# Mouafak-Khaled/Flow-Q-Learning

Hardware: AMD Instinct MI355X
Metric: FQL grad-steps/sec (whole node) over 16-α population, cube-single-v0 (higher is better)
Workload: dtype f32

## Files before the change

### flow-q-learning_amd/csrc/kernels.h

```cpp
#pragma once
#include <hip/hip_runtime.h>
#include <stdint.h>

namespace fq {

struct TRef {
    float* p;
    long long ss;
    long long sy;
};

inline TRef tref(float* p, long long ss, long long sy = 0) { return TRef{p, ss, sy}; }

enum GemmLayout { LAYOUT_FWD = 0, LAYOUT_DX = 1, LAYOUT_DW = 2 };
enum GemmEpi { EPI_STORE = 0, EPI_BIAS = 1, EPI_BIAS_GELU2 = 2, EPI_BIAS_GELU = 3, EPI_ADAM = 4 };

struct GemmArgs {
    TRef A, B, C, C2, bias;
    int M, N, K;
    int lda, ldb, ldc;
    int ny, nz;
    const int* slots;
    unsigned long long* probe;
};
void launch_gemm(int layout, int epi, int tile, const GemmArgs& a, hipStream_t s);
void launch_gemm_euler_hidden(const GemmArgs& a, hipStream_t s);
void launch_gemm_variant(int layout, int epi, int tile, int variant, const GemmArgs& a, hipStream_t s);
constexpr int GEMM_GROUP_MAX = 8;
struct Chunk { long long off; int len; int leaf; };
struct AdamArgs {
    const float* p_in;
    float* p_out;
    float *g, *m, *v;
    float* target;
    long long P, PT;
    long long net_off;
    const Chunk* chunks;
    const int* ids;
    int n_chunks, chunk_base;
    float* stats;
    int n_total_chunks;
    const int* count;
    float lr, tau;
    int nz;
    const int* slots;
};
struct AdamEpi {
    const float* p_in;
    float *p_out, *m, *v, *target, *wt_out;
    long long P, PT, PTT;
    long long ens, wt_sy;
    long long w_off[GEMM_GROUP_MAX];
    long long wt_off[GEMM_GROUP_MAX];
    int stat_base[GEMM_GROUP_MAX];
    float* stats;
    int n_total_chunks;
    const int* count;
    float lr, tau;
    int mode;
    int nt;
    AdamArgs small;
    int small_blocks;
};
struct GemmGroupArgs {
    GemmArgs g[GEMM_GROUP_MAX];
    int first[GEMM_GROUP_MAX + 1];
    int ng;
    AdamEpi adam;
};
void launch_gemm_group_dw(int tile, const GemmArgs* gs, int ng, hipStream_t s, const AdamEpi* adam = nullptr);
int gemm_group_tiles(int tile, int M, int N);

constexpr int EF_MAX_LAYERS = 8;
struct EulerArgs {
    const float* params;
    long long P;
    long long w_off[EF_MAX_LAYERS + 1];
    long long b_off[EF_MAX_LAYERS + 1];
    TRef eu;
    TRef aflow;
    int D, A, H, L, B, S, first;
    float steps_f;
    int nz;
    const int* slots;
    unsigned long long* probe;
    unsigned long long* phase;
};
constexpr int EF_PHASE_STRIDE = 4 * 10 * (EF_MAX_LAYERS + 1) + 8;
bool euler_flow_supported(int H, int L, int D, int A, int B);
void launch_euler_flow(const EulerArgs& a, hipStream_t s);

struct LnArgs {
    TRef u, h, mu, rstd, gamma, beta;
    int H, M, ld;
    int ny, nz;
    const int* slots;
};
void launch_ln_gelu_fwd(const LnArgs& a, hipStream_t s);

enum HeadMode { HEAD_STORE = 0, HEAD_BC_FUSED = 1, HEAD_EULER = 2, HEAD_OS = 3, HEAD_ACT = 4 };
struct HeadArgs {
    TRef h, W, b;
    TRef o0, o1, o2, o3;
    int H, M, ld, nout;
    int ld0, ld1, ld2, ld3;
    int B, D;
    int last;
    float steps_f;
    float t_next;
    int ny, nz;
    const int* slots;
};
void launch_head_fwd(int mode, const HeadArgs& a, hipStream_t s);

struct StreamArgs {
    const float* params;
    long long P, ens;
    long long w_off[EF_MAX_LAYERS + 1], b_off[EF_MAX_LAYERS + 1];
    long long g_off[EF_MAX_LAYERS], be_off[EF_MAX_LAYERS];
    const float* x0;
    long long x0_ss;
    int ld_x, K0, L, M;
    float* U[EF_MAX_LAYERS];
    float* G[EF_MAX_LAYERS];
    float* MU[EF_MAX_LAYERS];
    float* RS[EF_MAX_LAYERS];
    long long s_ss, s_sy, st_ss, st_sy;
    int ld_s, st_lo, st_hi;
    int g_hi;
    HeadArgs head;
    int ny, nz;
    const int* slots;
};
bool stream_fwd_supported(int H, int L, int K0, int nout, int M);
void launch_stream_fwd(int head_mode, bool ln, const StreamArgs& a, hipStream_t s);

struct SplitSync {
    unsigned long long* xch;
    unsigned* cnt;
    unsigned* gen;
    unsigned* err;
};
struct SplitFwdArgs {
    StreamArgs s;
    TRef aflow;
    int D, A, S, first;
    float steps_f;
    unsigned long long* probe;
    SplitSync sync;
    unsigned long long* phase;
    float* pre0;
};
long long split_cluster_bytes();
constexpr long long split_euler_pre0_floats() { return 2LL * 256 * 16; }
bool split_euler_pre0(int K0, int D);
int split_counter_stride();
bool split_fwd_supported(int H, int L, int K0, int nout, int M);
void launch_split_fwd(int head_mode, bool ln, bool euler, int F, const SplitFwdArgs& a, hipStream_t s);

struct StreamBwdArgs {
    const float* params;
    long long P, ens;
    const float* paramsT;
    long long PT, ensT;
    long long wt_off[EF_MAX_LAYERS];
    long long w_off[EF_MAX_LAYERS + 1], b_off[EF_MAX_LAYERS + 1];
    long long g_off[EF_MAX_LAYERS], be_off[EF_MAX_LAYERS];
    const float* dout;
    long long dout_ss, dout_sy;
    int ld_o;
    const float* U[EF_MAX_LAYERS];
    const float* Ghead;
    const float* MU[EF_MAX_LAYERS];
    const float* RS[EF_MAX_LAYERS];
    long long s_ss, s_sy, st_ss, st_sy;
    int ld_s, coff;
    float* DU[EF_MAX_LAYERS];
    long long d_ss, d_sy;
    int ld_d;
    float* part;
    int NP;
    int L, M, Mg, nout;
    float* da;
    long long da_ss, da_sy;
    int ld_da, D0, na;
    int ny, nz;
    const int* slots;
    unsigned long long* phase;
};
constexpr int SB_PHASE_STRIDE = 48;
bool stream_bwd_supported(int H, int L, int nout, int M, int Mg);
void launch_stream_bwd(bool ln, const StreamBwdArgs& a, hipStream_t s);
inline int stream_bwd_np(int L, int H, int nout, bool ln) { return (ln ? 3 : 1) * L * H + H * nout; }

bool split_bwd_supported(int H, int L, int nout, int M, int Mg);
void launch_split_bwd(bool ln, int F, const StreamBwdArgs& a, const SplitSync& sy, hipStream_t s);

struct ColsumArgs {
    const float* part;
    int NP, tiles;
    float* grads;
    long long P, ens;
    long long b_off[EF_MAX_LAYERS], g_off[EF_MAX_LAYERS], be_off[EF_MAX_LAYERS], w5_off;
    int L, H, ln;
    int ny, nz;
    const int* slots;
};
void launch_colsum_reduce(const ColsumArgs& a, hipStream_t s);

constexpr int TR_MAX = 32;
struct TransposeArgs {
    const float* src;
    long long src_ss;
    float* dst;
    long long dst_ss;
    long long src_off[TR_MAX], dst_off[TR_MAX];
    int n_mats, H;
    int nz;
    const int* slots;
};
void launch_transpose(const TransposeArgs& a, hipStream_t s);


struct BwdArgs {
    TRef dh;
    TRef dout, W5;
    TRef u, x_head;
    TRef mu, rstd, gamma;
    TRef c1, c2;
    TRef du;
    TRef g_b, g_gamma, g_beta, g_W5;
    int H, M, Mg, ld, ld_d, ld_o, nout;
    int ny, nz;
    const int* slots;
};
void launch_bwd_rowstats(bool head, const BwdArgs& a, hipStream_t s);
void launch_bwd_cols(bool head, bool ln, const BwdArgs& a, hipStream_t s);

struct InGradArgs {
    TRef W0, du0, da;
    int H, D, A, E, ld, off, M;
    int nz;
    const int* slots;
// ... 188 lines not shown
```

### flow-q-learning_amd/csrc/kernels.hip

```cpp
#include "kernels.h"

#include <hip/hip_runtime.h>
#include <math.h>

#include <type_traits>

#if defined(__HIP_DEVICE_COMPILE__) && !defined(__gfx950__)
#error "fqlpop kernels target gfx950 (MI355X) only: the s_waitcnt immediates use the gfx9 encoding"
#endif


namespace fq {

typedef float f32x16 __attribute__((ext_vector_type(16)));
typedef float f32x4 __attribute__((ext_vector_type(4)));

#define DEV __device__ __forceinline__

DEV float* at(TRef t, int slot, int y = 0) {
    return t.p + (long long)slot * t.ss + (long long)y * t.sy;
}

constexpr float kSqrt2OverPi = 0.7978845608028654f;

// ... 807 lines not shown
}

template <int EPI>
static void gemm_fwd_dma_dispatch(int tile, int stages, const GemmArgs& a, hipStream_t s) {
    auto grid = [&](int bm, int bn) { return dim3((a.M / bm) * (a.N / bn) * a.ny * a.nz); };
#define FQ_DMA(BM, BN, ST) hipLaunchKernelGGL((gemm_fwd_dma_kernel<BM, BN, ST, EPI>), grid(BM, BN), dim3(256), 0, s, a)
    if (tile == 0) {
        if (stages == 3) FQ_DMA(64, 64, 3);
        else FQ_DMA(64, 64, 4);
    } else if (tile == 1) {
        FQ_DMA(128, 64, 3);
    } else {
        FQ_DMA(64, 128, 3);
    }
#undef FQ_DMA
}

template <bool ARC, bool BRC, int EPI>
static void gemm_dispatch_tile(int tile, int variant, const GemmArgs& a, hipStream_t s) {
    if constexpr (!ARC && !BRC) {
        if (variant >= 4 && a.M % ((tile & 1) ? 128 : 64) == 0) {
            gemm_fwd_dma_dispatch<EPI>(tile, variant == 4 ? 3 : 4, a, s);
            return;
        }
    }
    variant &= 3;
    auto grid = [&](int bm, int bn) { return dim3(((a.M + bm - 1) / bm) * (a.N / bn) * a.ny * a.nz); };
    switch (tile) {
        case 0: gemm_dispatch_variant<64, 64, ARC, BRC, EPI>(variant, grid(64, 64), a, s); break;
        case 1: gemm_dispatch_variant<128, 64, ARC, BRC, EPI>(variant, grid(128, 64), a, s); break;
        case 2: gemm_dispatch_variant<64, 128, ARC, BRC, EPI>(variant, grid(64, 128), a, s); break;
        default: gemm_dispatch_variant<128, 128, ARC, BRC, EPI>(variant & 2, grid(128, 128), a, s); break;
    }
}

void launch_gemm_variant(int layout, int epi, int tile, int variant, const GemmArgs& a, hipStream_t s) {
    if ((tile & 2) && a.N % 128 != 0) tile &= ~2;
    if (layout != LAYOUT_FWD) variant &= 3;
    const int bk = (variant & 1) ? 64 : 32;
    if (layout != LAYOUT_FWD && a.K % bk != 0) variant &= ~1;
    if (layout == LAYOUT_FWD) {
        switch (epi) {
            case EPI_BIAS: gemm_dispatch_tile<false, false, EPI_BIAS>(tile, variant, a, s); break;
            case EPI_BIAS_GELU2: gemm_dispatch_tile<false, false, EPI_BIAS_GELU2>(tile, variant, a, s); break;
            default: gemm_dispatch_tile<false, false, EPI_BIAS_GELU>(tile, variant, a, s); break;
        }
    } else if (layout == LAYOUT_DX) {
        gemm_dispatch_tile<true, false, EPI_STORE>(tile, variant, a, s);
    } else {
        gemm_dispatch_tile<true, true, EPI_STORE>(tile, variant, a, s);
    }
}

void launch_gemm(int layout, int epi, int tile, const GemmArgs& a, hipStream_t s) {
    launch_gemm_variant(layout, epi, tile, 0, a, s);
}

void launch_gemm_euler_hidden(const GemmArgs& a, hipStream_t s) {
    const dim3 grid((a.M / 64) * (a.N / 64) * a.ny * a.nz);
    hipLaunchKernelGGL((gemm_fwd_dma_kernel<64, 64, 4, EPI_BIAS_GELU, 1>), grid, dim3(256), 0, s, a);
}

constexpr int EF_H = 512, EF_NC = 16, EF_NW = 8, EF_PF = 8, EF_K0MAX = 64;

constexpr float kG0 = -2.0f * 0.7978845608028654f * 1.4426950408889634f;
constexpr float kG1 = kG0 * 0.044715f;
DEV float gelu_sig(float x, float x2) {
    return __builtin_amdgcn_rcpf(1.0f + __builtin_amdgcn_exp2f(x * fmaf(x2, kG1, kG0)));
}
DEV float gelu_fast(float x) { return x * gelu_sig(x, x * x); }
constexpr float kD0 = 2.0f * 0.7978845608028654f, kD1 = kD0 * 3.0f * 0.044715f;
DEV void gelu_and_grad_fast(float x, float& g, float& gp) {
    const float x2 = x * x, sg = gelu_sig(x, x2);
    g = x * sg;
    gp = fmaf(sg, x * (1.0f - sg) * fmaf(x2, kD1, kD0), sg);
}
DEV float gelu_grad_fast(float x) {
    const float x2 = x * x, sg = gelu_sig(x, x2);
    return fmaf(sg, x * (1.0f - sg) * fmaf(x2, kD1, kD0), sg);
}

DEV void ln_acc(float v, float& s1, float& s2) {
#pragma clang fp contract(off)
    s1 = s1 + v;
    s2 = fmaf(v, v, s2);
}
DEV void ln_stats(float S1, float S2, float h, float& mean, float& rs) {
#pragma clang fp contract(off)
    mean = S1 / h;
    const float var = fmaxf(fmaf(-mean, mean, S2 / h), 0.f);
    rs = 1.0f / sqrtf(var + 1e-6f);
}
DEV float ln_apply(float v, float mean, float rs, float ga, float be) {
#pragma clang fp contract(off)
    return fmaf((v - mean) * rs, ga, be);
}
DEV float ln_bwd_acc(float dh, float gm, float xh, float& s1, float& s2) {
#pragma clang fp contract(off)
    const float d = dh * gm;
    s1 = s1 + d;
    s2 = fmaf(d, xh, s2);
    return d;
}
DEV float ln_bwd_du(float d, float xh, float c1, float c2, float rs, float gp) {
#pragma clang fp contract(off)
    return (rs * fmaf(-xh, c2, d - c1)) * gp;
}
DEV float mul_rn(float a, float b) {
#pragma clang fp contract(off)
    return a * b;
}

template <int PF = EF_PF>
DEV void ef_kloop(f32x4 (&acc)[4], float4 (&ring)[PF], rsrc_t rW, const float* xs, int NS, int w_cur,
                  int w_next, int lo, int lk, int li, int tail = -1) {
    constexpr int H = EF_H, NC = EF_NC;
    float bnext = xs[lk * NC + li];
    int s0 = 0;
    do {
        const int rbase = (s0 + PF < NS ? w_cur + 4 * (s0 + PF) * H : w_next) + lo;
        const int r0 = (s0 + PF >= NS && tail >= 0 ? tail : rbase - lo) + lo;
#pragma unroll
        for (int p = 0; p < PF; ++p) {
            const int s = s0 + p;
            const float b = bnext;
            bnext = xs[(4 * (s + 1) + lk) * NC + li];
            __builtin_amdgcn_sched_barrier(0);
            const float4 a = ring[p];
            acc[0] = __builtin_amdgcn_mfma_f32_16x16x4f32(a.x, b, acc[0], 0, 0, 0);
            acc[1] = __builtin_amdgcn_mfma_f32_16x16x4f32(a.y, b, acc[1], 0, 0, 0);
            acc[2] = __builtin_amdgcn_mfma_f32_16x16x4f32(a.z, b, acc[2], 0, 0, 0);
            acc[3] = __builtin_amdgcn_mfma_f32_16x16x4f32(a.w, b, acc[3], 0, 0, 0);
            __builtin_amdgcn_sched_barrier(0);
            ring[p] = bload4(rW, p == 0 ? r0 : rbase + 4 * p * H);
            __builtin_amdgcn_sched_barrier(0);
        }
        s0 += PF;
    } while (s0 < NS);
}

DEV void ef_tail(f32x4 (&acc)[4], float4 a, const float* xs, int lk, int li) {
    constexpr int NC = EF_NC;
    const float b = xs[(4 * EF_PF + lk) * NC + li];
    acc[0] = __builtin_amdgcn_mfma_f32_16x16x4f32(a.x, b, acc[0], 0, 0, 0);
    acc[1] = __builtin_amdgcn_mfma_f32_16x16x4f32(a.y, b, acc[1], 0, 0, 0);
    acc[2] = __builtin_amdgcn_mfma_f32_16x16x4f32(a.z, b, acc[2], 0, 0, 0);
    acc[3] = __builtin_amdgcn_mfma_f32_16x16x4f32(a.w, b, acc[3], 0, 0, 0);
}

bool euler_flow_supported(int H, int L, int D, int A, int B) {
    return H == EF_H && L >= 1 && L <= EF_MAX_LAYERS && D + A + 1 <= EF_K0MAX && A <= 8 && B % EF_NC == 0;
}

__global__ __launch_bounds__(EF_NW * 64, 1) void euler_flow_kernel(const EulerArgs g) {
    constexpr int H = EF_H, NC = EF_NC, NT = EF_NW * 64, PF = EF_PF;
    __shared__ __attribute__((aligned(16))) float slab[2][H * NC];
    __shared__ __attribute__((aligned(16))) float in0[EF_K0MAX * NC + 64];
    __shared__ float b5s[8];

    const int tiles = g.B / NC;
    const int total = tiles * g.nz;
    const int bid = xcd_remap(blockIdx.x, total);
    const int z = bid / tiles, c0 = (bid % tiles) * NC;
    const int slot = g.slots[z];
    const int tid = threadIdx.x, lane = tid & 63;
    const int w = __builtin_amdgcn_readfirstlane(tid >> 6);
    const int li = lane & 15, lk = lane >> 4;
    if (g.probe != nullptr && tid == 0) g.probe[2 * blockIdx.x] = __builtin_amdgcn_s_memrealtime();
#ifdef FQ_PHASE_PROBE
    unsigned long long* const ph = g.phase != nullptr ? g.phase + (long long)blockIdx.x * EF_PHASE_STRIDE : nullptr;
    auto stamp = [&](int i) {
        if (ph != nullptr && tid == 0) ph[i] = __builtin_amdgcn_s_memrealtime();
    };
#else
    auto stamp = [](int) {};
#endif
    stamp(0);

    const int D = g.D, A = g.A, L = g.L, B = g.B, S = g.S;
    const int K0 = D + A + 1;
#ifdef FQ_NO_EULER_TAIL
    const bool tail0 = false;
#else
    const bool tail0 = K0 > 4 * PF && K0 <= 4 * (PF + 1);
#endif
    const int NS0 = tail0 ? PF : (K0 + 4 * PF - 1) / (4 * PF) * PF;
    const float* __restrict__ P = g.params + (long long)slot * g.P;
    const float* __restrict__ eu = at(g.eu, slot);
    load_in0<NT>(in0, eu, D + A, B, c0);
    if (tid < A) b5s[tid] = P[g.b_off[L] + tid];
    const rsrc_t rW = make_rsrc(P, g.P);
    float w5r[16];
#pragma unroll
    for (int s = 0; s < 16; ++s) w5r[s] = bload1(rW, ((int)g.w_off[L] + (64 * w + 4 * s + lk) * A + li) * 4, 0);
#pragma unroll
    for (int s = 0; s < 16; ++s) w5r[s] = li < A ? w5r[s] : 0.f;

    const int lo = lk * H + 64 * w + 4 * li;
    float4 ring[PF];
#pragma unroll
    for (int p = 0; p < PF; ++p) ring[p] = bload4(rW, (int)g.w_off[0] + 4 * p * H + lo);
    __syncthreads();

    for (int step = g.first; step < S; ++step) {
        if (step == g.first) {
            if (tid < NC) in0[(D + A) * NC + tid] = (float)((double)step / (double)S);
            __syncthreads();
        }
        for (int l = 0; l < L; ++l) {
            const int NS = l == 0 ? NS0 : H / 4;
            const float* xs = l == 0 ? in0 : slab[(l - 1) & 1];
            float* xo = slab[l & 1];
            const int nl = l + 1 < L ? l + 1 : 0;
            f32x4 acc[4];
#pragma unroll
            for (int c = 0; c < 4; ++c) acc[c] = f32x4{0.f, 0.f, 0.f, 0.f};
            float4 bias4[4];
#pragma unroll
            for (int r = 0; r < 4; ++r) bias4[r] = bload4(rW, (int)g.b_off[l] + 64 * w + 16 * lk + 4 * r);
            __builtin_amdgcn_s_waitcnt(0x0F74);
            const int wcur = (int)g.w_off[l], wnext = (int)g.w_off[nl];
            asm volatile("" ::"s"(wcur), "s"(wnext));
            const int pi = 1 + 4 * ((step - g.first) * (L + 1) + l);
            stamp(pi);
            const bool tl = l == 0 && tail0;
            ef_kloop(acc, ring, rW, xs, NS, wcur, wnext, lo, lk, li, tl ? wcur + 4 * PF * H : -1);
            if (tl) {
                ef_tail(acc, ring[0], xs, lk, li);
                __builtin_amdgcn_sched_barrier(0);
                ring[0] = bload4(rW, wnext + lo);
            }
            stamp(pi + 1);
#pragma unroll
            for (int r = 0; r < 4; ++r) {
                const float bb[4] = {bias4[r].x, bias4[r].y, bias4[r].z, bias4[r].w};
#pragma unroll
                for (int c = 0; c < 4; ++c) {
                    const int f = 64 * w + 4 * (4 * lk + r) + c;
                    xo[f * NC + li] = gelu_fast(acc[c][r] + bb[c]);
                }
            }
            stamp(pi + 2);
            __syncthreads();
            stamp(pi + 3);
        }
        const int ph0 = 1 + 4 * ((step - g.first) * (L + 1) + L);
        stamp(ph0);
        float* red = slab[L & 1];
        {
            const float* hs = slab[(L - 1) & 1];
            f32x4 hacc = f32x4{0.f, 0.f, 0.f, 0.f};
#pragma unroll
            for (int s = 0; s < 16; ++s) {
                const int k = 64 * w + 4 * s + lk;
                hacc = __builtin_amdgcn_mfma_f32_16x16x4f32(w5r[s], hs[k * NC + li], hacc, 0, 0, 0);
            }
#pragma unroll
            for (int r = 0; r < 4; ++r) red[w * 16 * NC + (4 * lk + r) * NC + li] = hacc[r];
        }
        __syncthreads();
        if (tid < A * NC) {
            const int a = tid / NC, j = tid % NC;
            float v = red[tid];
#pragma unroll
            for (int q = 1; q < EF_NW; ++q) v += red[q * 16 * NC + tid];
            v += b5s[a];
            float* xp = &in0[(D + a) * NC + j];
            *xp = *xp + v / g.steps_f;
        } else if (tid < (A + 1) * NC && step + 1 < S) {
            in0[(D + A) * NC + tid - A * NC] = (float)((double)(step + 1) / (double)S);
        }
        __syncthreads();
        stamp(ph0 + 3);
    }
    if (tid < A * NC) {
        const int a = tid / NC, j = tid % NC;
        at(g.aflow, slot)[(long long)a * B + c0 + j] = clip1(in0[(D + a) * NC + j]);
    }
    if (g.probe != nullptr) {
        __syncthreads();
        if (tid == 0) g.probe[2 * blockIdx.x + 1] = __builtin_amdgcn_s_memrealtime();
    }
}

void launch_euler_flow(const EulerArgs& a, hipStream_t s) {
    const dim3 grid((a.B / EF_NC) * a.nz);
    hipLaunchKernelGGL(euler_flow_kernel, grid, dim3(EF_NW * 64), 0, s, a);
}

constexpr int CW = 16;

#define FQ_KPT_DISPATCH(H, KERNEL, ...)                                      \
    switch ((H) / CW) {                                                      \
        case 4: KERNEL(4, __VA_ARGS__); break;                               \
        case 8: KERNEL(8, __VA_ARGS__); break;                               \
        case 16: KERNEL(16, __VA_ARGS__); break;                             \
        case 32: KERNEL(32, __VA_ARGS__); break;                             \
        default: KERNEL(64, __VA_ARGS__); break;                             \
    }

template <int KPT>
__global__ __launch_bounds__(1024) void ln_gelu_fwd_kernel(const LnArgs a) {
    const int ncb = a.M / 64;
    const int cb = blockIdx.x % ncb, yz = blockIdx.x / ncb;
    const int y = yz % a.ny, z = yz / a.ny;
    const int slot = a.slots[z];
    const int lane = threadIdx.x & 63;
    const int w = __builtin_amdgcn_readfirstlane(threadIdx.x >> 6);
    const int m = cb * 64 + lane;
    const long long ld = a.ld;
    const float* __restrict__ u = at(a.u, slot, y) + m;
    const int k0 = w * KPT;
    float g[KPT];
#pragma unroll
    for (int i = 0; i < KPT; ++i) g[i] = u[(k0 + i) * ld];
    float s1 = 0.f, s2 = 0.f;
#pragma unroll
    for (int i = 0; i < KPT; ++i) {
        g[i] = gelu_f(g[i]);
        s1 += g[i];
        s2 += g[i] * g[i];
    }
    __shared__ float red[2][CW][64];
    red[0][w][lane] = s1;
    red[1][w][lane] = s2;
    __syncthreads();
    float S1 = 0.f, S2 = 0.f;
#pragma unroll
    for (int q = 0; q < CW; ++q) {
        S1 += red[0][q][lane];
        S2 += red[1][q][lane];
    }
    const float mean = S1 / (float)a.H;
    const float var = fmaxf(S2 / (float)a.H - mean * mean, 0.f);
    const float rs = 1.0f / sqrtf(var + 1e-6f);
    float* __restrict__ h = at(a.h, slot, y) + m;
    const float* __restrict__ gam = at(a.gamma, slot, y) + k0;
    const float* __restrict__ bet = at(a.beta, slot, y) + k0;
#pragma unroll
    for (int i = 0; i < KPT; ++i) h[(k0 + i) * ld] = (g[i] - mean) * rs * gam[i] + bet[i];
    if (w == 0) {
        at(a.mu, slot, y)[m] = mean;
        at(a.rstd, slot, y)[m] = rs;
    }
}

#define FQ_LN_LAUNCH(KPT, grid, s, a) hipLaunchKernelGGL(ln_gelu_fwd_kernel<KPT>, grid, dim3(1024), 0, s, a)
void launch_ln_gelu_fwd(const LnArgs& a, hipStream_t s) {
    const dim3 grid((a.M / 64) * a.ny * a.nz);
    FQ_KPT_DISPATCH(a.H, FQ_LN_LAUNCH, grid, s, a)
}

template <int MODE>
DEV void head_write(const HeadArgs& a, int slot, int y, int j, int m, float v) {
    const int B = a.B, D = a.D;
    if constexpr (MODE == HEAD_STORE) {
        at(a.o0, slot, y)[(long long)j * a.ld0 + m] = v;
    } else if constexpr (MODE == HEAD_ACT) {
        at(a.o0, slot, y)[(long long)j * a.ld0 + m] = clip1(v);
    } else if constexpr (MODE == HEAD_BC_FUSED) {
        if (m < B) {
            at(a.o0, slot)[(long long)j * a.ld0 + m] = v;
        } else {
            const int mm = m - B;
            const float x = at(a.o1, slot)[(long long)(D + j) * a.ld1 + m];
            float* eu = at(a.o2, slot);
            eu[(long long)(D + j) * a.ld2 + mm] = x + v / a.steps_f;
            if (j == 0) eu[(long long)(D + a.nout) * a.ld2 + mm] = a.t_next;
        }
    } else if constexpr (MODE == HEAD_EULER) {
        float* eu = at(a.o2, slot);
        const long long o = (long long)(D + j) * a.ld2 + m;
        const float xn = eu[o] + v / a.steps_f;
        if (a.last) {
            at(a.o0, slot)[(long long)j * a.ld0 + m] = clip1(xn);
        } else {
            eu[o] = xn;
            if (j == 0) eu[(long long)(D + a.nout) * a.ld2 + m] = a.t_next;
        }
    } else if constexpr (MODE == HEAD_OS) {
        if (m < B) {
            at(a.o1, slot)[(long long)(D + j) * a.ld1 + m] = clip1(v);
        } else if (m < 2 * B) {
            const int mm = m - B;
            at(a.o0, slot)[(long long)j * a.ld0 + mm] = v;
            at(a.o2, slot)[(long long)(D + j) * a.ld2 + B + mm] = clip1(v);
        } else {
            at(a.o3, slot)[(long long)j * a.ld3 + (m - 2 * B)] = clip1(v);
        }
    }
}

template <int MODE, int KPT>
__global__ __launch_bounds__(1024) void head_fwd_kernel(const HeadArgs a) {
    const int ncb = a.M / 64;
    const int cb = blockIdx.x % ncb, yz = blockIdx.x / ncb;
    const int y = yz % a.ny, z = yz / a.ny;
    const int slot = a.slots[z];
    const int lane = threadIdx.x & 63;
    const int w = __builtin_amdgcn_readfirstlane(threadIdx.x >> 6);
    const int m = cb * 64 + lane;
    const long long ld = a.ld;
    const int nout = a.nout;
    const int k0 = w * KPT;
    const float* __restrict__ h = at(a.h, slot, y) + m;
    const float* __restrict__ W = at(a.W, slot, y) + (long long)k0 * nout;
    float hv[KPT];
#pragma unroll
    for (int i = 0; i < KPT; ++i) hv[i] = h[(k0 + i) * ld];
    float acc[8];
#pragma unroll
    for (int j = 0; j < 8; ++j) acc[j] = 0.f;
#pragma unroll
    for (int i = 0; i < KPT; ++i)
#pragma unroll
        for (int j = 0; j < 8; ++j)
            if (j < nout) acc[j] += W[i * nout + j] * hv[i];
    __shared__ float red[CW][8][64];
#pragma unroll
    for (int j = 0; j < 8; ++j) red[w][j][lane] = acc[j];
    __syncthreads();
    const int t = threadIdx.x;
    if (t < nout * 64) {
        const int j = t >> 6, l2 = t & 63;
        float v = 0.f;
#pragma unroll
        for (int q = 0; q < CW; ++q) v += red[q][j][l2];
        v += at(a.b, slot, y)[j];
        head_write<MODE>(a, slot, y, j, cb * 64 + l2, v);
    }
}

#define FQ_HEAD_LAUNCH(KPT, MODE, grid, s, a) \
    hipLaunchKernelGGL((head_fwd_kernel<MODE, KPT>), grid, dim3(1024), 0, s, a)
void launch_head_fwd(int mode, const HeadArgs& a, hipStream_t s) {
    const dim3 grid((a.M / 64) * a.ny * a.nz);
    switch (mode) {
        case HEAD_STORE: FQ_KPT_DISPATCH(a.H, FQ_HEAD_LAUNCH, HEAD_STORE, grid, s, a) break;
        case HEAD_BC_FUSED: FQ_KPT_DISPATCH(a.H, FQ_HEAD_LAUNCH, HEAD_BC_FUSED, grid, s, a) break;
        case HEAD_EULER: FQ_KPT_DISPATCH(a.H, FQ_HEAD_LAUNCH, HEAD_EULER, grid, s, a) break;
// ... 2897 lines not shown
```

### flow-q-learning_amd/csrc/runtime.cpp

```cpp
#include <hip/hip_runtime.h>

#include <algorithm>
#include <cmath>
#include <cstdio>
#include <cstdlib>
#include <cstring>
#include <functional>
#include <map>
#include <set>
#include <memory>
#include <string>
#include <vector>

#include "../../include/fqlpop.h"
#include "kernels.h"

using namespace fq;

namespace {

thread_local std::string g_err;

struct FqErr {
    int code;
    std::string msg;
};

#define HIPCHK(x)                                                                                 \
    do {                                                                                          \
        hipError_t e_ = (x);                                                                      \
        if (e_ != hipSuccess)                                                                     \
            throw FqErr{FQLPOP_E_HIP, std::string(#x) + " failed: " + hipGetErrorString(e_)};     \
    } while (0)

#define ARGCHK(c, m)                                         \
    do {                                                     \
        if (!(c)) throw FqErr{FQLPOP_E_ARG, std::string(m)}; \
    } while (0)

constexpr long long kAlign = 64;
long long align_up(long long x) { return (x + kAlign - 1) / kAlign * kAlign; }

#ifdef FQ_DIAG
const char* diag_env(const char* name) { return std::getenv(name); }
#else
const char* diag_env(const char*) { return nullptr; }
#endif

struct EngineOptions {
    int euler_fused = 1;
    int stream_fwd = 1;
    int stream_bwd = 1;
    int fused_adam = 1;
    int serial = 0;
    int dw_tile_critic = 10, dw_tile_actor = 10;
    int adam_nt = 3;
    int split = 1;
    int small_sched = 1;
    int split_blocks = 256;
    int split_sites = 0;
    int hw_queues = 4;
    int em_seq_sweep = 1;
    int em_ens_xcd = 0;
};
EngineOptions g_engine_opts;

constexpr int kStepBranches = 4;
int step_streams(const EngineOptions& eo) {
    return (eo.serial || eo.hw_queues < kStepBranches) ? 1 : kStepBranches;
}

struct EngineOptionRef {
    const char* name;
    int EngineOptions::*field;
    int lo, hi;
};
const EngineOptionRef kEngineOptions[] = {
    {"euler_fused", &EngineOptions::euler_fused, 0, 1}, {"stream_fwd", &EngineOptions::stream_fwd, 0, 1},
    {"stream_bwd", &EngineOptions::stream_bwd, 0, 1},   {"fused_adam", &EngineOptions::fused_adam, 0, 1},
    {"serial", &EngineOptions::serial, 0, 1},
    {"dw_tile_critic", &EngineOptions::dw_tile_critic, 0, 10},
    {"dw_tile_actor", &EngineOptions::dw_tile_actor, 0, 10},
    {"adam_nt", &EngineOptions::adam_nt, 0, 3},
    {"split", &EngineOptions::split, 0, 8},
    {"small_sched", &EngineOptions::small_sched, 0, 1},
    {"hw_queues", &EngineOptions::hw_queues, 1, 1024},
    {"split_sites", &EngineOptions::split_sites, 0, (1 << 24) - 1},
    {"split_blocks", &EngineOptions::split_blocks, 64, 1024},
    {"em_seq_sweep", &EngineOptions::em_seq_sweep, 0, 1},
    {"em_ens_xcd", &EngineOptions::em_ens_xcd, 0, 1},
};

void philox_host(uint32_t c[4], uint32_t k0, uint32_t k1) {
    for (int r = 0; r < 10; ++r) {
        const uint64_t p0 = (uint64_t)0xD2511F53u * c[0], p1 = (uint64_t)0xCD9E8D57u * c[2];
        const uint32_t hi0 = (uint32_t)(p0 >> 32), lo0 = (uint32_t)p0;
        const uint32_t hi1 = (uint32_t)(p1 >> 32), lo1 = (uint32_t)p1;
        const uint32_t n0 = hi1 ^ c[1] ^ k0, n2 = hi0 ^ c[3] ^ k1;
        c[0] = n0; c[1] = lo1; c[2] = n2; c[3] = lo0;
        k0 += 0x9E3779B9u;
        k1 += 0xBB67AE85u;
    }
}

uint64_t sample_key(uint64_t seed, float alpha) {
    uint32_t ab;
    std::memcpy(&ab, &alpha, sizeof(ab));
    uint64_t z = seed ^ ((uint64_t)ab << 32 | 0x9E3779B9u);
    z = (z ^ (z >> 30)) * 0xBF58476D1CE4E5B9ull;
    z = (z ^ (z >> 27)) * 0x94D049BB133111EBull;
    return z ^ (z >> 31);
}

struct NetLayout {
    std::string name;
    int in_dim = 0, out_dim = 0, L = 0, H = 0, E = 1;
    bool ln = false;
    long long off = 0;
    long long ens_size = 0;
    std::vector<long long> W, b, gam, bet;
    int kdim(int l) const { return l == 0 ? in_dim : H; }
    int ndim(int l) const { return l == L ? out_dim : H; }

    void build(const std::string& nm, int in, int out, int nh, int h, int e, bool use_ln) {
        name = nm; in_dim = in; out_dim = out; L = nh; H = h; E = e; ln = use_ln;
        long long o = 0;
        for (int l = 0; l <= L; ++l) {
            W.push_back(o); o = align_up(o + (long long)kdim(l) * ndim(l));
            b.push_back(o); o = align_up(o + ndim(l));
            if (l < L && ln) {
                gam.push_back(o); o = align_up(o + H);
                bet.push_back(o); o = align_up(o + H);
            }
        }
        ens_size = o;
    }
    long long size() const { return ens_size * E; }
};

struct Leaf {
    std::string name;
    int net;
    int kind;
    int layer;
    int ndim;
    long long shape[3];
    long long flat_off;
    long long size;
};

struct Graphs {
    hipGraphExec_t exec = nullptr;
    int nz = -1;
};

struct Buf {
    float* p = nullptr;
    long long ss = 0;
    TRef ref(long long sy = 0) const { return TRef{p, ss, sy}; }
    TRef cols(long long off, long long sy = 0) const { return TRef{p + off, ss, sy}; }
};

struct Net {
    const NetLayout* lay = nullptr;
    float* const* arena = nullptr;
    long long arena_ss = 0;
    int ni = 0;
    const Buf* X = nullptr;
    int ld = 0;
    int ld_d = 0, ld_o = 0;
    long long sy = 0, st_sy = 0;
    bool keep_u = true;
    bool dominant = false;
    std::vector<Buf> U, G, MU, RS, DU;
    Buf DH, C1, C2, part;
    int fwd_site = -1, bwd_site = -1;
    int skip_fwd = 0, skip_bwd = 0;
    TRef par(long long off) const { return tref(*arena + lay->off + off, arena_ss, lay->ens_size); }
    TRef act(const Buf& b, long long coff = 0) const { return b.cols(coff, sy); }
    TRef stat(const Buf& b, long long coff = 0) const { return b.cols(coff, st_sy); }
    TRef grad(const Buf& b) const { return b.ref((long long)lay->H * ld_d); }
};

}

struct fqlpop {
    fqlpop_config cfg{};
    EngineOptions opt{};
    int n = 0;
    int device = 0;
    int D = 0, A = 0, H = 0, L = 0, B = 0, E = 0, S = 0;
    NetLayout critic, bc, os;
    long long P = 0, PT = 0;
    std::vector<Leaf> leaves;
    long long state_size = 0;

    float* params_buf[2] = {nullptr, nullptr};
    Buf paramsT_buf[2];
    int cur = 0;
    float *params = nullptr, *params_nx = nullptr;
    float *grads = nullptr, *adam_m = nullptr, *adam_v = nullptr, *target = nullptr;
    int* count = nullptr;
    uint64_t* seeds = nullptr;
    uint64_t* skeys = nullptr;
    float* alpha = nullptr;
    int* slots = nullptr;
    float* stats = nullptr;
    Chunk* chunks = nullptr;
    int* chunk_leaf = nullptr;
    int* leaf_first = nullptr;
    int n_chunks_net[3] = {0, 0, 0}, chunk_base_net[3] = {0, 0, 0}, n_chunks_total = 0;
    bool fused_adam = false;
    int w_stat_base[3][EF_MAX_LAYERS] = {};
    int* res_ids = nullptr;
    int res_base[3] = {0, 0, 0}, res_n[3] = {0, 0, 0};
    int n_train_leaves = 0;

    std::vector<float> h_alpha;
    std::vector<uint64_t> h_seeds;
    std::vector<uint8_t> active;
    std::vector<int> h_slots;
    int nz = 0;

    struct Dataset {
        float *obs = nullptr, *act = nullptr, *rew = nullptr, *mask = nullptr, *nobs = nullptr;
        long long rows = 0;
    } ds[2];

    std::vector<float*> allocs;
    Buf os_in, bc_in, eu_in, cr_in, tg_in;
    Buf cr_in_buf[2];
    Net n_cr, n_tg, n_bc, n_eu, n_os;
    Buf q, qt, dq, vpred, dv, act_t, x0_t, rew_t, mask_t, apiraw, aflow, amet, da, dout_os;
// ... 576 lines not shown
            ae.w_off[gi] = N.off + N.W[l];
            ae.wt_off[gi] = l >= 1 ? h->wt_net_off[ni] + (long long)(l - 1) * N.H * N.H : -1;
            ae.stat_base[gi] = h->w_stat_base[ni][l];
        }
        ae.stats = h->stats; ae.n_total_chunks = h->n_chunks_total;
        ae.count = h->count;
        ae.lr = h->cfg.lr; ae.tau = h->cfg.tau;
        {
            const char* dm = diag_env("FQLPOP_DW_MODE");
            ae.mode = dm ? std::atoi(dm) : 0;
            if (ae.mode == 4) ae.mode = ni == 0 ? 0 : 3;
            ae.nt = h->opt.adam_nt;
        }
        ae.small = adam_args(c, ni);
        ae.small_blocks = ae.small.n_chunks * c.nz;
        launch_gemm_group_dw(dw_tile(h, N), gs.data(), (int)gs.size(), sw, &ae);
    } else if (N.L <= GEMM_GROUP_MAX && N.H % 128 == 0) {
        launch_gemm_group_dw(dw_tile(h, N), gs.data(), (int)gs.size(), sw);
    } else {
        for (const GemmArgs& gw : gs) gemm(LAYOUT_DW, EPI_STORE, gw, sw);
    }
    };
    if (defer) *defer = dw_half;
    else dw_half();
}

void transpose_nets(fqlpop* h, hipStream_t s, int mask, bool all_slots, const float* src, const Buf& dst) {
    TransposeArgs t{};
    t.src = src; t.src_ss = h->P;
    t.dst = dst.p; t.dst_ss = dst.ss;
    t.H = h->H;
    const NetLayout* nets[3] = {&h->critic, &h->bc, &h->os};
    const long long HH = (long long)h->H * h->H;
    int n = 0;
    for (int ni = 0; ni < 3; ++ni) {
        if (!(mask & (1 << ni))) continue;
        const NetLayout& N = *nets[ni];
        for (int e = 0; e < N.E; ++e)
            for (int l = 1; l < N.L; ++l) {
                ARGCHK(n < TR_MAX, "too many transposed matrices");
                t.src_off[n] = N.off + e * N.ens_size + N.W[l];
                t.dst_off[n] = h->wt_net_off[ni] + ((long long)e * (N.L - 1) + (l - 1)) * HH;
                ++n;
            }
    }
    t.n_mats = n;
    if (all_slots) { t.slots = nullptr; t.nz = h->n; }
    else { t.slots = h->slots; t.nz = h->nz; }
    launch_transpose(t, s);
}

AdamArgs adam_args(const Ctx& c, int ni) {
    fqlpop* h = c.h;
    const NetLayout* nets[3] = {&h->critic, &h->bc, &h->os};
    AdamArgs a{};
    a.p_in = h->params; a.p_out = h->params_nx;
    a.g = h->grads; a.m = h->adam_m; a.v = h->adam_v;
    a.target = ni == 0 ? h->target : nullptr;
    a.P = h->P; a.PT = h->PT;
    a.net_off = nets[ni]->off;
    a.chunks = h->chunks;
    if (h->fused_adam) {
        a.ids = h->res_ids + h->res_base[ni];
        a.n_chunks = h->res_n[ni];
    } else {
        a.ids = nullptr;
        a.n_chunks = h->n_chunks_net[ni];
        a.chunk_base = h->chunk_base_net[ni];
    }
    a.stats = h->stats; a.n_total_chunks = h->n_chunks_total;
    a.count = h->count;
    a.lr = h->cfg.lr; a.tau = h->cfg.tau;
    a.nz = c.nz; a.slots = h->slots;
    return a;
}

void adam_net(const Ctx& c, hipStream_t s, int ni) {
    const AdamArgs a = adam_args(c, ni);
    if (a.n_chunks > 0) launch_adam(a, s);
}

struct FwdCols {
    int st_lo, st_hi;
    int g_hi = -1;
};

void stream_fwd(const Ctx& c, hipStream_t s, const Net& n, const FwdCols& k, int mode, const HeadArgs& head) {
    fqlpop* h = c.h;
    const NetLayout& N = *n.lay;
    const bool store = k.st_hi > k.st_lo, stats = store && !n.MU.empty();
    StreamArgs a{};
    a.params = *n.arena + N.off;
    a.P = n.arena_ss;
    a.ens = N.ens_size;
    for (int l = 0; l <= N.L; ++l) {
        a.w_off[l] = N.W[l];
        a.b_off[l] = N.b[l];
        if (l < N.L && N.ln) {
            a.g_off[l] = N.gam[l];
            a.be_off[l] = N.bet[l];
        }
        if (l < N.L && store) {
            a.U[l] = n.U[l].p;
            a.G[l] = n.G[l].p;
            if (stats && N.ln) { a.MU[l] = n.MU[l].p; a.RS[l] = n.RS[l].p; }
        }
    }
    a.x0 = n.X->p;
    a.x0_ss = n.X->ss;
    a.ld_x = n.ld; a.K0 = N.in_dim; a.L = N.L; a.M = n.ld;
    if (store) { a.s_ss = n.U[0].ss; a.s_sy = n.sy; }
    if (stats) { a.st_ss = n.MU[0].ss; a.st_sy = n.st_sy; }
    a.ld_s = n.ld; a.st_lo = k.st_lo; a.st_hi = k.st_hi;
    a.g_hi = k.g_hi < 0 ? k.st_hi : k.g_hi;
    a.head = head;
    a.head.nout = N.out_dim;
    a.ny = N.E; a.nz = c.nz; a.slots = h->slots;
    if (skip_mask() & n.skip_fwd) return;
    const int F = c.plan.F[n.fwd_site];
    if (F > 1) {
        SplitFwdArgs sa{};
        sa.s = a;
        sa.sync = split_prep(h, n.fwd_site, (long long)(n.ld / 16) * N.E * c.nz, s);
        launch_split_fwd(mode, N.ln, false, F, sa, s);
    } else {
        launch_stream_fwd(mode, N.ln, a, s);
    }
}

long long euler_blocks(const Ctx& c) { return (long long)(c.h->B / 16) * c.nz * c.plan.F[SITE_EULER]; }
SplitFwdArgs euler_split_args(const Ctx& c, const EulerArgs& ea, hipStream_t s) {
    fqlpop* h = c.h;
    const NetLayout& N = h->bc;
    SplitFwdArgs sa{};
    StreamArgs& a = sa.s;
    a.params = ea.params; a.P = ea.P; a.ens = 0;
    for (int l = 0; l <= N.L; ++l) { a.w_off[l] = ea.w_off[l]; a.b_off[l] = ea.b_off[l]; }
    a.x0 = ea.eu.p; a.x0_ss = ea.eu.ss; a.ld_x = ea.B; a.K0 = ea.D + ea.A + 1; a.L = ea.L; a.M = ea.B;
    a.head.nout = ea.A;
    a.ny = 1; a.nz = ea.nz; a.slots = ea.slots;
    sa.aflow = ea.aflow;
    sa.D = ea.D; sa.A = ea.A; sa.S = ea.S; sa.first = ea.first; sa.steps_f = ea.steps_f;
    sa.probe = ea.probe;
    sa.phase = ea.phase;
    sa.sync = split_prep(h, SITE_EULER, (long long)(ea.B / 16) * ea.nz, s);
    sa.pre0 = h->euler_pre0 && euler_blocks(c) <= h->euler_pre0_blocks ? h->euler_pre0 : nullptr;
    return sa;
}
void launch_euler(const Ctx& c, const EulerArgs& ea, hipStream_t s) {
    const int F = c.plan.F[SITE_EULER];
    ARGCHK(ea.probe == nullptr || euler_blocks(c) <= c.h->probe_blocks, "Euler probe: too many blocks");
    ARGCHK(ea.phase == nullptr || euler_blocks(c) <= c.h->ephase_blocks, "Euler phase probe: too many blocks");
    if (F > 1) launch_split_fwd(HEAD_EULER, false, true, F, euler_split_args(c, ea, s), s);
    else launch_euler_flow(ea, s);
}

int skip_mask() {
    static const int m = [] { const char* v = diag_env("FQLPOP_SKIP"); return v ? std::atoi(v) : 0; }();
    return m;
}

EulerArgs euler_args(fqlpop* h, int nz) {
    const NetLayout& N = h->bc;
    EulerArgs ea{};
    ea.params = h->params + N.off;
    ea.P = h->P;
    for (int l = 0; l <= N.L; ++l) {
        ea.w_off[l] = N.W[l];
        ea.b_off[l] = N.b[l];
    }
    ea.eu = h->eu_in.ref();
    ea.aflow = h->aflow.ref();
    ea.D = h->D; ea.A = h->A; ea.H = h->H; ea.L = h->L; ea.B = h->B; ea.S = h->S; ea.first = 1;
    ea.steps_f = (float)h->S;
    ea.nz = nz; ea.slots = h->slots;
    ea.phase = h->ephase_dev;
    return ea;
}

double dominant_flops(const fqlpop* h) {
    const double B = h->B, H = h->H, K0 = h->D + h->A + 1, A = h->A;
    if (h->euler_fused)
        return (h->S - 1) * 2.0 * B * (K0 * H + (h->L - 1) * H * H + H * A) * h->nz;
    return 2.0 * H * B * H * h->nz;
}

void phase_report(const unsigned long long* ph, long long nb, int L, bool ln, const char* name) {
    long long t0 = -1, t1 = 0, n = 0;
    double blk = 0, pro = 0, tail = 0, pass1[8] = {}, wait2[8] = {}, p2[8] = {}, prod[8] = {}, hp[4] = {};
    for (long long b = 0; b < nb; ++b) {
        const unsigned long long* p = ph + b * SB_PHASE_STRIDE;
        if (p[0] == 0 || p[1] < p[0]) continue;
        ++n;
        t0 = t0 < 0 ? (long long)p[0] : std::min(t0, (long long)p[0]);
        t1 = std::max(t1, (long long)p[1]);
        blk += (double)(p[1] - p[0]);
        pro += (double)(p[2] - p[0]);
        tail += (double)(p[1] - p[2 + 5 * (L - 1) + 3]);
        if (p[40] != 0)
            for (int i = 0; i < 4; ++i) hp[i] += (double)(p[40 + i] - (i == 0 ? p[0] : p[39 + i]));
        for (int i = 0; i < L && i < 8; ++i) {
            const unsigned long long* q = p + 2 + 5 * i;
            if (ln) {
                pass1[i] += (double)(q[1] - q[0]);
                wait2[i] += (double)(q[2] - q[1]);
                p2[i] += (double)(q[3] - q[2]);
            } else {
                p2[i] += (double)(q[3] - q[0]);
            }
            if (i + 1 < L) prod[i] += (double)(q[4] - q[3]);
        }
    }
    if (n == 0) return;
    const double us = 0.01 / (double)n;
    std::fprintf(stderr,
                 "phase probe (%s backward, last launch): %lld blocks, span %.1f us, block %.2f us "
                 "(prologue %.2f, after the last slab barrier %.2f)\n",
                 name, n, (double)(t1 - t0) * 0.01, blk * us, pro * us, tail * us);
    if (hp[0] > 0)
        std::fprintf(stderr, "  prologue: head operands staged %.2f | barrier %.2f | head grads %.2f | dh + barrier %.2f\n",
                     hp[0] * us, hp[1] * us, hp[2] * us, hp[3] * us);
    for (int i = 0; i < L && i < 8; ++i)
        if (ln)
            std::fprintf(stderr, "  pass %d: LN pass 1 %.2f | stats barrier %.2f | pass 2 + du + slab barrier %.2f | dX product %.2f\n",
                         i, pass1[i] * us, wait2[i] * us, p2[i] * us, prod[i] * us);
        else
            std::fprintf(stderr, "  pass %d: GELU' + du + slab barrier (+ dQ/da at pass %d) %.2f | dX product %.2f\n",
                         i, L - 1, p2[i] * us, prod[i] * us);
}

void euler_phase_report(const unsigned long long* ph, long long nb, int L, int steps) {
    double kl[9] = {}, ep[9] = {}, br[9] = {}, gap[9] = {}, pro = 0, blk = 0;
    long long n = 0;
    for (long long b = 0; b < nb; ++b) {
        const unsigned long long* p = ph + b * EF_PHASE_STRIDE;
        if (p[0] == 0) continue;
        ++n;
        pro += (double)(p[1] - p[0]);
        blk += (double)(p[1 + 4 * ((steps - 1) * (L + 1) + L) + 3] - p[0]);
        for (int st = 0; st < steps; ++st)
            for (int l = 0; l <= L; ++l) {
                const unsigned long long* q = p + 1 + 4 * (st * (L + 1) + l);
                if (l < L) {
                    kl[l] += (double)(q[1] - q[0]);
                    ep[l] += (double)(q[2] - q[1]);
                    br[l] += (double)(q[3] - q[2]);
                    gap[l] += (double)(q[0] - (l > 0 ? q[-1] : st > 0 ? q[-1] : q[0]));
                } else {
                    kl[l] += (double)(q[3] - q[0]);
                }
            }
    }
    if (n == 0) return;
    const double us = 0.01 / (double)n, per = us / (double)steps;
    std::fprintf(stderr, "phase probe (Euler flow, last launch): %lld blocks, %d steps, block %.1f us, prologue %.2f us\n",
                 n, steps, blk * us, pro * us);
    for (int l = 0; l < L; ++l)
        std::fprintf(stderr, "  layer %d per step: k-loop %.3f | epilogue %.3f | barrier %.3f | gap before %.3f\n", l,
                     kl[l] * per, ep[l] * per, br[l] * per, gap[l] * per);
    std::fprintf(stderr, "  head per step: %.3f\n", kl[L] * per);
}

void split_euler_phase_report(const unsigned long long* ph, long long nb, int L, int steps) {
    double stg[9] = {}, kl[9] = {}, ep[9] = {}, head = 0, pro = 0, blk = 0, l0 = 0;
    long long n = 0, t0 = -1, t1 = 0, tl = 0;
    int xcc[8] = {};
    for (long long b = 0; b < nb; ++b) {
        const unsigned long long* p = ph + b * EF_PHASE_STRIDE;
        if (p[0] == 0) continue;
        ++n;
        t0 = t0 < 0 ? (long long)p[0] : std::min(t0, (long long)p[0]);
        tl = std::max(tl, (long long)p[0]);
        const unsigned long long* e = p + 1 + 4 * ((steps - 1) * (L + 1) + L);
        t1 = std::max(t1, (long long)e[3]);
        pro += (double)(p[1] - p[0]);
        blk += (double)(e[3] - p[0]);
        ++xcc[p[EF_PHASE_STRIDE - 1] & 7];
        for (int st = 0; st < steps; ++st) {
            const unsigned long long* q0 = p + 1 + 4 * (st * (L + 1));
            l0 += (double)(q0[3] - q0[0]);
            for (int l = 1; l < L; ++l) {
                const unsigned long long* q = q0 + 4 * l;
                stg[l] += (double)(q[1] - q[0]);
                kl[l] += (double)(q[2] - q[1]);
                ep[l] += (double)(q[3] - q[2]);
            }
            const unsigned long long* qh = q0 + 4 * L;
            head += (double)(qh[3] - qh[0]);
        }
    }
    if (n == 0) return;
    const double us = 0.01 / (double)n, per = us / (double)steps;
    std::fprintf(stderr, "phase probe (split Euler flow, last launch): %lld blocks, %d steps, span %.1f us, block %.1f us, "
                 "start spread %.2f us, prologue %.2f us; blocks per XCC %d %d %d %d %d %d %d %d\n",
                 n, steps, (double)(t1 - t0) * 0.01, blk * us, (double)(tl - t0) * 0.01, pro * us, xcc[0], xcc[1],
                 xcc[2], xcc[3], xcc[4], xcc[5], xcc[6], xcc[7]);
    std::fprintf(stderr, "  layer 0 per step (redundant, no hand-off): %.3f\n", l0 * per);
    for (int l = 1; l < L; ++l)
        std::fprintf(stderr, "  layer %d per step: stage (wait + copy) %.3f | k-loop %.3f | epilogue + publish %.3f\n", l,
                     stg[l] * per, kl[l] * per, ep[l] * per);
    std::fprintf(stderr, "  head per step (wait for the 8 partials + update): %.3f\n", head * per);
}

void flip_params(fqlpop* h);

void enqueue(fqlpop* h, bool train, bool inj_batch, bool inj_noise) {
    const Ctx c = step_ctx(h);
// ... 1875 lines not shown
```

Measured before the change: 8295.

## Overlap Euler flow layer epilogue with next layer's first K-half via wave handoff

Adds a paired variant of the fused Euler-flow kernel. The upper half of the waves delay their GELU epilogue until after the block barrier, and each hidden layer's K-loop is split into two halves. The second half spins on a workgroup-shared counter until the late waves have written their outputs. This overlaps epilogue writes with the next layer's MFMA work, replacing part of the barrier stall with a spin-wait on a shared atomic, at the cost of ordering subtleties and a bounded spin.

New measurement: 7991. 3.7% lower.

```diff
diff --git a/flow-q-learning_amd/csrc/kernels.h b/flow-q-learning_amd/csrc/kernels.h
--- a/flow-q-learning_amd/csrc/kernels.h
+++ b/flow-q-learning_amd/csrc/kernels.h
@@ -88,7 +88,7 @@
 };
 constexpr int EF_PHASE_STRIDE = 4 * 10 * (EF_MAX_LAYERS + 1) + 8;
 bool euler_flow_supported(int H, int L, int D, int A, int B);
-void launch_euler_flow(const EulerArgs& a, hipStream_t s);
+void launch_euler_flow(const EulerArgs& a, bool pair, hipStream_t s);
 
 struct LnArgs {
     TRef u, h, mu, rstd, gamma, beta;
diff --git a/flow-q-learning_amd/csrc/kernels.hip b/flow-q-learning_amd/csrc/kernels.hip
--- a/flow-q-learning_amd/csrc/kernels.hip
+++ b/flow-q-learning_amd/csrc/kernels.hip
@@ -983,11 +983,13 @@
     return H == EF_H && L >= 1 && L <= EF_MAX_LAYERS && D + A + 1 <= EF_K0MAX && A <= 8 && B % EF_NC == 0;
 }
 
+template <bool PAIR>
 __global__ __launch_bounds__(EF_NW * 64, 1) void euler_flow_kernel(const EulerArgs g) {
     constexpr int H = EF_H, NC = EF_NC, NT = EF_NW * 64, PF = EF_PF;
     __shared__ __attribute__((aligned(16))) float slab[2][H * NC];
     __shared__ __attribute__((aligned(16))) float in0[EF_K0MAX * NC + 64];
     __shared__ float b5s[8];
+    __shared__ int handoff;
 
     const int tiles = g.B / NC;
     const int total = tiles * g.nz;
@@ -997,6 +999,7 @@
     const int tid = threadIdx.x, lane = tid & 63;
     const int w = __builtin_amdgcn_readfirstlane(tid >> 6);
     const int li = lane & 15, lk = lane >> 4;
+    const bool late = PAIR && w >= EF_NW / 2;
     if (g.probe != nullptr && tid == 0) g.probe[2 * blockIdx.x] = __builtin_amdgcn_s_memrealtime();
 #ifdef FQ_PHASE_PROBE
     unsigned long long* const ph = g.phase != nullptr ? g.phase + (long long)blockIdx.x * EF_PHASE_STRIDE : nullptr;
@@ -1020,6 +1023,7 @@
     const float* __restrict__ eu = at(g.eu, slot);
     load_in0<NT>(in0, eu, D + A, B, c0);
     if (tid < A) b5s[tid] = P[g.b_off[L] + tid];
+    if (PAIR && tid == 0) handoff = 0;
     const rsrc_t rW = make_rsrc(P, g.P);
     float w5r[16];
 #pragma unroll
@@ -1032,6 +1036,21 @@
 #pragma unroll
     for (int p = 0; p < PF; ++p) ring[p] = bload4(rW, (int)g.w_off[0] + 4 * p * H + lo);
     __syncthreads();
+
+    f32x4 acc[4];
+    float4 bias4[4];
+    auto epilogue = [&](float* xo) {
+#pragma unroll
+        for (int r = 0; r < 4; ++r) {
+            const float bb[4] = {bias4[r].x, bias4[r].y, bias4[r].z, bias4[r].w};
+#pragma unroll
+            for (int c = 0; c < 4; ++c) {
+                const int f = 64 * w + 4 * (4 * lk + r) + c;
+                xo[f * NC + li] = gelu_fast(acc[c][r] + bb[c]);
+            }
+        }
+    };
+    int handoffs = 0;
 
     for (int step = g.first; step < S; ++step) {
         if (step == g.first) {
@@ -1043,10 +1062,8 @@
             const float* xs = l == 0 ? in0 : slab[(l - 1) & 1];
             float* xo = slab[l & 1];
             const int nl = l + 1 < L ? l + 1 : 0;
-            f32x4 acc[4];
 #pragma unroll
             for (int c = 0; c < 4; ++c) acc[c] = f32x4{0.f, 0.f, 0.f, 0.f};
-            float4 bias4[4];
 #pragma unroll
             for (int r = 0; r < 4; ++r) bias4[r] = bload4(rW, (int)g.b_off[l] + 64 * w + 16 * lk + 4 * r);
             __builtin_amdgcn_s_waitcnt(0x0F74);
@@ -1055,25 +1072,42 @@
             const int pi = 1 + 4 * ((step - g.first) * (L + 1) + l);
             stamp(pi);
             const bool tl = l == 0 && tail0;
-            ef_kloop(acc, ring, rW, xs, NS, wcur, wnext, lo, lk, li, tl ? wcur + 4 * PF * H : -1);
+            if (!PAIR) {
+                ef_kloop(acc, ring, rW, xs, NS, wcur, wnext, lo, lk, li, tl ? wcur + 4 * PF * H : -1);
+            } else {
+                const int nh = l == 0 ? 1 : 2, NSh = l == 0 ? NS : H / 8;
+#pragma unroll 1
+                for (int h = 0; h < nh; ++h) {
+                    if (h == 1) {
+                        __atomic_signal_fence(__ATOMIC_SEQ_CST);
+                        for (int spin = 0; spin < (1 << 22); ++spin)
+                            if (__builtin_amdgcn_readfirstlane(__hip_atomic_load(&handoff, __ATOMIC_RELAXED, __HIP_MEMORY_SCOPE_WORKGROUP)) >= handoffs) break;
+                        __atomic_signal_fence(__ATOMIC_SEQ_CST);
+                    }
+                    const int wc = wcur + h * (H / 2) * H;
+                    ef_kloop(acc, ring, rW, xs + h * (H / 2) * NC, NSh, wc, h + 1 < nh ? wc + (H / 2) * H : wnext, lo, lk, li,
+                             tl ? wcur + 4 * PF * H : -1);
+                }
+            }
             if (tl) {
                 ef_tail(acc, ring[0], xs, lk, li);
                 __builtin_amdgcn_sched_barrier(0);
                 ring[0] = bload4(rW, wnext + lo);
             }
             stamp(pi + 1);
-#pragma unroll
-            for (int r = 0; r < 4; ++r) {
-                const float bb[4] = {bias4[r].x, bias4[r].y, bias4[r].z, bias4[r].w};
-#pragma unroll
-                for (int c = 0; c < 4; ++c) {
-                    const int f = 64 * w + 4 * (4 * lk + r) + c;
-                    xo[f * NC + li] = gelu_fast(acc[c][r] + bb[c]);
-                }
-            }
+            if (!late) epilogue(xo);
             stamp(pi + 2);
             __syncthreads();
             stamp(pi + 3);
+            if (PAIR) {
+                if (late) {
+                    epilogue(xo);
+                    __atomic_signal_fence(__ATOMIC_SEQ_CST);
+                    if (lane == 0) __hip_atomic_fetch_add(&handoff, 1, __ATOMIC_RELAXED, __HIP_MEMORY_SCOPE_WORKGROUP);
+                    __atomic_signal_fence(__ATOMIC_SEQ_CST);
+                }
+                handoffs += EF_NW / 2;
+            }
         }
         const int ph0 = 1 + 4 * ((step - g.first) * (L + 1) + L);
         stamp(ph0);
@@ -1114,9 +1148,10 @@
     }
 }
 
-void launch_euler_flow(const EulerArgs& a, hipStream_t s) {
+void launch_euler_flow(const EulerArgs& a, bool pair, hipStream_t s) {
     const dim3 grid((a.B / EF_NC) * a.nz);
-    hipLaunchKernelGGL(euler_flow_kernel, grid, dim3(EF_NW * 64), 0, s, a);
+    if (pair) hipLaunchKernelGGL(euler_flow_kernel<true>, grid, dim3(EF_NW * 64), 0, s, a);
+    else hipLaunchKernelGGL(euler_flow_kernel<false>, grid, dim3(EF_NW * 64), 0, s, a);
 }
 
 constexpr int CW = 16;
diff --git a/flow-q-learning_amd/csrc/runtime.cpp b/flow-q-learning_amd/csrc/runtime.cpp
--- a/flow-q-learning_amd/csrc/runtime.cpp
+++ b/flow-q-learning_amd/csrc/runtime.cpp
@@ -49,6 +49,7 @@
 
 struct EngineOptions {
     int euler_fused = 1;
+    int euler_pair = 1;
     int stream_fwd = 1;
     int stream_bwd = 1;
     int fused_adam = 1;
@@ -78,7 +79,7 @@
 const EngineOptionRef kEngineOptions[] = {
     {"euler_fused", &EngineOptions::euler_fused, 0, 1}, {"stream_fwd", &EngineOptions::stream_fwd, 0, 1},
     {"stream_bwd", &EngineOptions::stream_bwd, 0, 1},   {"fused_adam", &EngineOptions::fused_adam, 0, 1},
-    {"serial", &EngineOptions::serial, 0, 1},
+    {"serial", &EngineOptions::serial, 0, 1},           {"euler_pair", &EngineOptions::euler_pair, 0, 1},
     {"dw_tile_critic", &EngineOptions::dw_tile_critic, 0, 10},
     {"dw_tile_actor", &EngineOptions::dw_tile_actor, 0, 10},
     {"adam_nt", &EngineOptions::adam_nt, 0, 3},
@@ -961,7 +962,7 @@
     ARGCHK(ea.probe == nullptr || euler_blocks(c) <= c.h->probe_blocks, "Euler probe: too many blocks");
     ARGCHK(ea.phase == nullptr || euler_blocks(c) <= c.h->ephase_blocks, "Euler phase probe: too many blocks");
     if (F > 1) launch_split_fwd(HEAD_EULER, false, true, F, euler_split_args(c, ea, s), s);
-    else launch_euler_flow(ea, s);
+    else launch_euler_flow(ea, c.h->opt.euler_pair != 0, s);
 }
 
 int skip_mask() {
```
